# pandekan/tomography_alignment

Hardware: AMD Instinct MI355X
Metric: sirt_iterations_per_sec (higher is better)
Workload: dtype f32

## Files before the change

tomography_alignment_amd/csrc/kernels_tile_gather.hip.h:

```cpp

#define GTX 8
#define GTY 8
#define GROWS 14
#define GPITCH 68
#ifndef GWAVES
#define GWAVES 4
#endif
#ifndef GPX
#define GPX 8
#define GPY 12
#endif

struct GfC {
    int64_t fp0x, fp0y, fux, fuy, fdx, fdy;
    float m00, m01, m10, m11;
    float p0x, p0y, tau;
    int32_t n, zc, slot;
};

__global__ __launch_bounds__(256) void k_sino_zflags(const float *__restrict__ proj, long long n_rows, int ndz, unsigned char *__restrict__ flags)
{
    const int iz = (int)(blockIdx.x * 256 + threadIdx.x);
    if (iz >= ndz) return;
    bool nz = false;
    for (long long r = blockIdx.y; r < n_rows; r += gridDim.y) nz |= proj[(size_t)r * ndz + iz] != 0.f;
    if (nz) flags[iz] = 1;
}

__global__ __launch_bounds__(1024) void k_zflags_prefix(const unsigned char *__restrict__ flags, int n, int *__restrict__ cum)
{
    __shared__ int wsum[16];
    __shared__ int base;
    const int lane = threadIdx.x & 63, wv = threadIdx.x >> 6;
    if (threadIdx.x == 0) base = 0;
    __syncthreads();
    for (int i0 = 0; i0 < n; i0 += 1024) {
        const int i = i0 + (int)threadIdx.x;
        const bool f = i < n && flags[i] != 0;
        const unsigned long long m = __builtin_amdgcn_ballot_w64(f);
        if (lane == 0) wsum[wv] = (int)__builtin_popcountll(m);
        __syncthreads();
        int off = base;
        for (int w = 0; w < wv; ++w) off += wsum[w];
        if (i < n) cum[i] = off + (int)__builtin_popcountll(m & ((1ull << lane) - 1ull));
        __syncthreads();
        if (threadIdx.x == 0) {
            int t = 0;
            for (int w = 0; w < 16; ++w) t += wsum[w];
            base += t;
        }
        __syncthreads();
    }
    if (threadIdx.x == 0) cum[n] = base;
}

__global__ __launch_bounds__(64) void k_zchunk_shift(const unsigned char *__restrict__ flags, int ndz, int nz, int zc_lo, int zc_hi, int *__restrict__ shift)
{
    const int n_chunk = (nz + 63) / 64;
    int first = n_chunk;
    for (int c = threadIdx.x; c < n_chunk; c += 64) {
        bool any = false;
        for (int i = max(0, 64 * c - zc_hi - 1); i <= min(ndz - 1, 64 * c + 63 - zc_lo) && !any; ++i) any = flags[i] != 0;
        if (any) first = min(first, c);
    }
#pragma unroll
    for (int o = 32; o > 0; o >>= 1) first = min(first, __shfl_xor(first, o, 64));
    if (threadIdx.x == 0) *shift = first >= n_chunk ? 0 : (GWAVES - first % GWAVES) % GWAVES;
}

template <bool ZERO>
__device__ __forceinline__ void gather_update_store(float *__restrict__ dst, const float *__restrict__ vv, const float *__restrict__ gt, const f32x2 (&acc2)[32],
                                                    int z0, int nz, int positivity, double *__restrict__ err_out)
{
    double err = 0.0;
#define G_UPD1(R, A, V, G)                                  \
    {                                                       \
        float pr_ = (A) * (V);                              \
        asm volatile("" : "+v"(pr_));        \
        R = R + pr_;                                        \
        if (positivity && R < 0.f) R = 0.f;                 \
        if (gt) { const float e_ = (G) - R; err += (double)e_ * (double)e_; } \
    }
    if (z0 + 64 <= nz && (nz & 3) == 0) {
#pragma unroll
        for (int p = 0; p < 64; p += 4) {
            float4 r = *(float4 *)(dst + p);
            const float4 v = *(const float4 *)(vv + p);
            float4 t = {0.f, 0.f, 0.f, 0.f};
            if (gt) t = *(const float4 *)(gt + p);
            G_UPD1(r.x, ZERO ? 0.f : acc2[p / 2].x, v.x, t.x)
            G_UPD1(r.y, ZERO ? 0.f : acc2[p / 2].y, v.y, t.y)
            G_UPD1(r.z, ZERO ? 0.f : acc2[p / 2 + 1].x, v.z, t.z)
            G_UPD1(r.w, ZERO ? 0.f : acc2[p / 2 + 1].y, v.w, t.w)
            *(float4 *)(dst + p) = r;
            __builtin_amdgcn_sched_barrier(0);
        }
    } else {
#pragma unroll
        for (int p = 0; p < 64; ++p)
            if (z0 + p < nz) {
                float r = dst[p];
                G_UPD1(r, ZERO ? 0.f : ((p & 1) ? acc2[p / 2].y : acc2[p / 2].x), vv[p], gt[p])
                dst[p] = r;
            }
    }
#undef G_UPD1
    if (gt) {
        err = wave_sum_d(err);
        if ((threadIdx.x & 63) == 0) atomicAdd(err_out, err);
    }
}

template <int NJ, int UPD>
__global__ __launch_bounds__(GWAVES * 64, 16 / GWAVES) void k_adj_gather_flat(const GfC *__restrict__ cs, int n_proj, const float *__restrict__ proj,
                                                                 float *__restrict__ vol, TomoGeomC g, int xs, int xe, int patched,
                                                                 const unsigned char *__restrict__ zflags, int zc_lo, int zc_hi, const int *__restrict__ zshift,
                                                                 const float *__restrict__ upd_v, const float *__restrict__ upd_gt, int positivity,
                                                                 double *__restrict__ upd_err)
{
    __shared__ __attribute__((aligned(16))) float rows[GWAVES][GROWS * GPITCH];
    __shared__ float4 wtab[3][GWAVES][64];
    const int lane = threadIdx.x & 63;
    const int wv = __builtin_amdgcn_readfirstlane(threadIdx.x >> 6);
    const int ntx = (xe - xs + GTX - 1) / GTX, nty = (g.ny + GTY - 1) / GTY, nzq = (g.nz + 64 * GWAVES - 1) / (64 * GWAVES) + 1;
    int tx, ty, zq;
    if (patched) {
        const int npx = (ntx + GPX - 1) / GPX, npy = (nty + GPY - 1) / GPY;
        const int slot = (int)(blockIdx.x >> 3), patch = (slot / (GPX * GPY)) * 8 + (int)(blockIdx.x & 7), within = slot % (GPX * GPY);
        const int pxy = patch % (npx * npy);
        zq = patch / (npx * npy);
        tx = (pxy / npy) * GPX + within / GPY;
        ty = (pxy % npy) * GPY + within % GPY;
    } else {
        zq = (int)(blockIdx.x % (unsigned)nzq);
        ty = (int)((blockIdx.x / (unsigned)nzq) % (unsigned)nty);
        tx = (int)(blockIdx.x / ((unsigned)nzq * (unsigned)nty));
    }
    const int x0 = xs + tx * GTX, y0 = ty * GTY, z0 = (zq * GWAVES + wv - *zshift) * 64;
    if (tx >= ntx || ty >= nty || zq >= nzq) return;
    bool zlive = z0 >= 0 && z0 < g.nz;
    if (zlive) {
        bool any = false;
        for (int i = z0 - zc_hi - 1 + lane; i <= z0 + 63 - zc_lo; i += 64) any |= i >= 0 && i < g.ndz && zflags[i] != 0;
        zlive = __builtin_amdgcn_ballot_w64(any) != 0;
    }
    __shared__ int wlive[GWAVES];
    if (lane == 0) wlive[wv] = zlive ? 1 : 0;
    __syncthreads();
    int nl = 0, rk = 0;
#pragma unroll
    for (int w = 0; w < GWAVES; ++w) { nl += wlive[w]; rk += w < wv ? wlive[w] : 0; }
#if !defined(__gfx950__) && !defined(__gfx942__) && !defined(__gfx90a__) && defined(__HIP_DEVICE_COMPILE__)
#error "k_adj_gather_flat: divergent exit before barriers is only known to be safe on gfx9-family targets (s_barrier ignores ended waves)"
#endif
    if (UPD && !zlive && z0 >= 0 && z0 < g.nz && (positivity || upd_gt)) {
        const int X = x0 + (lane >> 3), Y = y0 + (lane & 7);
        if (X < xe && Y < g.ny) {
            const size_t o = ((size_t)X * g.ny + Y) * g.nz + z0;
            f32x2 none[32];
            gather_update_store<true>(vol + o, upd_v + o, upd_gt ? upd_gt + o : nullptr, none, z0, g.nz, positivity, upd_err);
        }
    }
    if (!zlive) return;
    const int X = x0 + (lane >> 3), Y = y0 + (lane & 7), Zl = z0 + lane;
    float *wrows = rows[wv];
    const size_t n_det = (size_t)g.ndx * g.ndz;
    const uint32_t pitch4 = (uint32_t)g.ndz * 4u;
    const float two_m32 = 2.3283064365386963e-10f;
    f32x2 acc2[32];
#pragma unroll
    for (int p = 0; p < 32; ++p) acc2[p] = f32x2{0.f, 0.f};

#define G_TABLE(IPX, BUF, SLOT)                                                                                            \
    {                                                                                                                      \
        float4 t4 = {0.f, 0.f, 0.f, 0.f};                                                                                  \
        if ((IPX) < n_proj) {                                                                                              \
            const GfC &ct = cs[IPX];                                                                                       \
            const float qx = (float)X - ct.p0x, qy = (float)Y - ct.p0y;                                                    \
            const float a = ct.m00 * qx + ct.m01 * qy, b = ct.m10 * qx + ct.m11 * qy;                                      \
            const int i0 = (int)ceilf(a - (fabsf(ct.m00) + fabsf(ct.m01) + 5e-3f));                                        \
            const int j0 = (int)ceilf(b - (fabsf(ct.m10) + fabsf(ct.m11) + 5e-3f));                                        \
            int64_t rx = ct.fp0x + (int64_t)i0 * ct.fux + (int64_t)j0 * ct.fdx - ((int64_t)X << 32);                       \
            int64_t ry = ct.fp0y + (int64_t)i0 * ct.fuy + (int64_t)j0 * ct.fdy - ((int64_t)Y << 32);                       \
            float W[3];                                                                                                    \
            _Pragma("unroll") for (int k = 0; k < 3; ++k) {                                                                \
                int64_t sx = rx, sy = ry;                                                                                  \
                float wsum = 0.f;                                                                                          \
                _Pragma("unroll") for (int mth = 0; mth < NJ; ++mth) {                                                     \
                    const int hx = (int)(sx >> 32), hy = (int)(sy >> 32);                                                  \
                    const float fx = (float)(unsigned)sx * two_m32, fy = (float)(unsigned)sy * two_m32;                    \
                                                        \
                    const float wx = select_lanes2(select_lanes(fx, __builtin_amdgcn_ballot_w64(hx == -1)), 1.f - fx, __builtin_amdgcn_ballot_w64(hx == 0)); \
                    const float wy = select_lanes2(select_lanes(fy, __builtin_amdgcn_ballot_w64(hy == -1)), 1.f - fy, __builtin_amdgcn_ballot_w64(hy == 0)); \
                    wsum += select_lanes(wx * wy, __builtin_amdgcn_ballot_w64((unsigned)(j0 + mth) < (unsigned)ct.n));     \
                    sx += ct.fdx; sy += ct.fdy;                                                                            \
                }                                                                                                          \
                W[k] = select_lanes(wsum, __builtin_amdgcn_ballot_w64((unsigned)(i0 + k) < (unsigned)g.ndx));              \
                rx += ct.fux; ry += ct.fuy;                                                                                \
            }                                                                                                              \
            t4.x = __builtin_bit_cast(float, i0); t4.y = W[0]; t4.z = W[1]; t4.w = W[2];                                   \
        }                                                                                                                  \
        wtab[BUF][SLOT][lane] = t4;                                                                                        \
    }
    float4 tn;
    int ix_lo_n;
    float y0v[GROWS], yedge = 0.f;
#ifdef TOMO_ABLATE_GATHER_LOADS
#define G_ROW_LOAD(P) __int_as_float(0x3f800000 + (int)(size_t)(P))
#else
#define G_ROW_LOAD(P) (*(const float *)(P))
#endif
#define G_SETUP(IPX, BUF, SLOT)                                                                                            \
    {                                                                                                                      \
        tn = wtab[BUF][SLOT][lane];                                                                                        \
        const int i0s = __builtin_bit_cast(int, tn.x);                                                                     \
        ix_lo_n = __builtin_amdgcn_readfirstlane(wave_min_i32(i0s));                                                       \
        if (zlive) {                                                                                                       \
            const GfC &cn = cs[IPX];                                                                                       \
            const int iz0 = Zl - cn.zc;                                                                                    \
            const char *srow = (const char *)(proj + (size_t)cn.slot * n_det);                           \
             \
             \
             \
             \
            const uint32_t o0 = (uint32_t)min(max(iz0, 0), g.ndz - 1) * 4u;                                                 \
            const uint32_t rowoff = (uint32_t)min(max(ix_lo_n + min(lane, GROWS - 1), 0), g.ndx - 1) * pitch4;              \
            _Pragma("unroll") for (int r = 0; r < GROWS; ++r)                                                              \
                y0v[r] = G_ROW_LOAD(srow + (o0 + (uint32_t)__builtin_amdgcn_readlane((int)rowoff, r)));                     \
             \
             \
            if (cn.tau != 0.f) {                                             \
                const uint32_t oe = (uint32_t)min(max(z0 - cn.zc - 1, 0), g.ndz - 1) * 4u;                                  \
                yedge = *(const float *)(srow + (rowoff + oe));                                                            \
            }                                                                                                              \
        }                                                                                                                  \
    }
    const int n_grp = (n_proj + nl - 1) / nl;
    int buf = 0;
    if (n_grp > 0) {
        G_TABLE(rk, 0, rk)
        __syncthreads();
        G_SETUP(0, 0, 0)
    }
    for (int grp = 0; grp < n_grp; ++grp) {
        const int nbuf = buf == 2 ? 0 : buf + 1;
        if (grp + 1 < n_grp) G_TABLE((grp + 1) * nl + rk, nbuf, rk)
        __syncthreads();
        const int g0 = grp * nl, g1 = min(n_proj, g0 + nl);
        for (int ip = g0; ip < g1; ++ip) {
            const GfC &c = cs[ip];
            const float4 t = tn;
            const int i0 = __builtin_bit_cast(int, t.x), ix_lo = ix_lo_n;
            const float W0 = t.y, W1 = t.z, W2 = t.w;
            const bool hit = zlive && __any(W0 != 0.f || W1 != 0.f || W2 != 0.f);
            if (hit) {
                const int iz0 = Zl - c.zc, iz1 = iz0 - 1;
                const unsigned long long m0 = __builtin_amdgcn_ballot_w64(iz0 >= 0) & __builtin_amdgcn_ballot_w64(iz0 < g.ndz);
                const unsigned long long m1 = __builtin_amdgcn_ballot_w64(iz1 >= 0) & __builtin_amdgcn_ballot_w64(iz1 < g.ndz);
#define G_ZLERP(MASKED)                                                                                                           \
    _Pragma("unroll") for (int r = 0; r < GROWS; ++r) {                                                                           \
        float y1 = dpp_shr1_f(y0v[r]);                                             \
        asm("v_writelane_b32 %0, %1, 0" : "+v"(y1) : "s"(__builtin_amdgcn_readlane(__builtin_bit_cast(int, yedge), r)));    \
        const float a0 = (MASKED) ? select_lanes(y0v[r], m0) : y0v[r], a1 = (MASKED) ? select_lanes(y1, m1) : y1;                \
        wrows[r * GPITCH + lane] = fmaf(c.tau, a1 - a0, a0);                                                                      \
    }
                if (c.tau == 0.f) {
                    if (m0 == ~0ull) {
#pragma unroll
                        for (int r = 0; r < GROWS; ++r) wrows[r * GPITCH + lane] = y0v[r];
                    } else {
#pragma unroll
                        for (int r = 0; r < GROWS; ++r) wrows[r * GPITCH + lane] = select_lanes(y0v[r], m0);
                    }
                }
                else if ((m0 & m1) == ~0ull) { G_ZLERP(false) }
                else { G_ZLERP(true) }
#undef G_ZLERP
            }
            if (ip + 1 < g1) G_SETUP(ip + 1, buf, ip + 1 - g0)
            else if (ip + 1 < n_proj) G_SETUP(ip + 1, nbuf, 0)
            if (hit) {
                const int slot0 = min(max(i0 - ix_lo, 0), GROWS - 3);
                const float4 *q = (const float4 *)__builtin_assume_aligned(wrows + slot0 * GPITCH, 16);
                float4 n0 = q[0], n1 = q[GPITCH / 4], n2 = q[2 * GPITCH / 4];
#pragma unroll
                for (int p = 0; p < 64; p += 4) {
                    const float4 r0 = n0, r1 = n1, r2 = n2;
                    if (p + 4 < 64) { n0 = q[(p + 4) / 4]; n1 = q[(GPITCH + p + 4) / 4]; n2 = q[(2 * GPITCH + p + 4) / 4]; }
                    acc2[p / 2] = W2 * f32x2{r2.x, r2.y} + (W1 * f32x2{r1.x, r1.y} + (W0 * f32x2{r0.x, r0.y} + acc2[p / 2]));
                    acc2[p / 2 + 1] = W2 * f32x2{r2.z, r2.w} + (W1 * f32x2{r1.z, r1.w} + (W0 * f32x2{r0.z, r0.w} + acc2[p / 2 + 1]));
                    __builtin_amdgcn_sched_barrier(0);
                }
            }
        }
        buf = nbuf;
    }
#undef G_TABLE
#undef G_SETUP
    if (UPD) {
        if (X < xe && Y < g.ny) {
            const size_t o = ((size_t)X * g.ny + Y) * g.nz + z0;
            gather_update_store<false>(vol + o, upd_v + o, upd_gt ? upd_gt + o : nullptr, acc2, z0, g.nz, positivity, upd_err);
        }
    } else if (zlive && X < xe && Y < g.ny) {
        float *dst = vol + ((size_t)X * g.ny + Y) * g.nz + z0;
        if (z0 + 64 <= g.nz && (g.nz & 3) == 0) {
#pragma unroll
            for (int p = 0; p < 64; p += 4) {
                float4 v = *(float4 *)(dst + p);
                v.x += acc2[p / 2].x; v.y += acc2[p / 2].y; v.z += acc2[p / 2 + 1].x; v.w += acc2[p / 2 + 1].y;
                *(float4 *)(dst + p) = v;
            }
        } else {
#pragma unroll
            for (int p = 0; p < 64; ++p)
                if (z0 + p < g.nz) dst[p] += (p & 1) ? acc2[p / 2].y : acc2[p / 2].x;
        }
    }
}


#define FGROWS 24
#define FG_NONE (1 << 29)

template <int NW, int WALKY>
__device__ __forceinline__ void fwd_gather_flat_body(const GfC *__restrict__ cs, const int *__restrict__ perm, int n_list, unsigned block_id,
                                                     float *__restrict__ proj, const float *__restrict__ vol, const TomoGeomC &g,
                                                     const unsigned char *__restrict__ vflags, const int *__restrict__ zshift,
                                                     float (*rows)[FGROWS * GPITCH], float4 (*wtab)[GWAVES][64], int (*ltab)[GWAVES][64], int *wlive)
{
    static_assert(NW == 3 || NW == 4, "NW");
    constexpr int SW = FGROWS - NW + 1;
    const int lane = threadIdx.x & 63;
    const int wv = __builtin_amdgcn_readfirstlane(threadIdx.x >> 6);
    const int nS = WALKY ? g.ny : g.nx, nL = WALKY ? g.nx : g.ny;
    const uint32_t strideL4 = (WALKY ? (uint32_t)g.ny * (uint32_t)g.nz : (uint32_t)g.nz) * 4u;
    const size_t strideS = WALKY ? (size_t)g.nz : (size_t)g.ny * g.nz;
    const int npg = (n_list + 7) / 8, nrt = (g.ndx + 7) / 8, nzq = (g.nz + 64 * GWAVES - 1) / (64 * GWAVES) + 1;
    const int m_all = npg * nrt, m8 = (m_all + 7) / 8;
    const int slot_id = (int)(block_id >> 3), xcd = (int)(block_id & 7);
    const int zq = slot_id / m8, tile = xcd * m8 + slot_id % m8;
    if (tile >= m_all || zq >= nzq) return;
    const int pg = tile / nrt, rt = tile % nrt;
    const int z0 = (zq * GWAVES + wv - *zshift) * 64;
    bool zlive = z0 >= 0 && z0 < g.nz;
    if (zlive) {
        const int i = z0 + lane;
        zlive = __builtin_amdgcn_ballot_w64(i < g.nz && vflags[i] != 0) != 0;
    }
    if (lane == 0) wlive[wv] = zlive ? 1 : 0;
    __syncthreads();
    int nl = 0, rk = 0;
#pragma unroll
    for (int w = 0; w < GWAVES; ++w) { nl += wlive[w]; rk += w < wv ? wlive[w] : 0; }
#if !defined(__gfx950__) && !defined(__gfx942__) && !defined(__gfx90a__) && defined(__HIP_DEVICE_COMPILE__)
#error "k_fwd_gather_flat: divergent exit before barriers is only known to be safe on gfx9-family targets (s_barrier ignores ended waves)"
#endif
    if (!zlive) return;

    const int ipl = pg * 8 + (lane >> 3), ix = rt * 8 + (lane & 7);
    const int pe = perm[min(ipl, n_list - 1)];
    const bool ray_ok = ipl < n_list && ix < g.ndx && pe >= 0;
    const GfC &c = cs[max(pe, 0)];
    const int64_t fds = WALKY ? c.fdy : c.fdx, fdl = WALKY ? c.fdx : c.fdy;
    const int64_t bs0 = (WALKY ? c.fp0y : c.fp0x) + (int64_t)ix * (WALKY ? c.fuy : c.fux);
    const int64_t bl0 = (WALKY ? c.fp0x : c.fp0y) + (int64_t)ix * (WALKY ? c.fux : c.fuy);
    const float bsf = (float)((double)bs0 * 2.3283064365386963e-10), inv_ds = (float)(4294967296.0 / (double)fds);
    const int n_smp = ray_ok ? c.n : 0;
    const float two_m32 = 2.3283064365386963e-10f;
    const int Zl = z0 + lane;
    const unsigned long long mz = __builtin_amdgcn_ballot_w64(Zl < g.nz);
    const uint32_t o0 = (uint32_t)min(Zl, g.nz - 1) * 4u;
    float *wrows = rows[wv];
    f32x2 acc2[32];
#pragma unroll
    for (int p = 0; p < 32; ++p) acc2[p] = f32x2{0.f, 0.f};

#define FG_TABLE(SX, BUF, SLOT)                                                                                            \
    {                                                                                                                      \
        float W[4] = {0.f, 0.f, 0.f, 0.f};                                                                                 \
        int L0 = FG_NONE;                                                                                                  \
        if ((SX) < nS) {                                                                                                   \
            const float ta = ((float)((SX) - 1) - bsf) * inv_ds, tb = ((float)((SX) + 1) - bsf) * inv_ds;                  \
            const int j0 = (int)ceilf(fminf(ta, tb) - 5e-3f);                                                              \
            int64_t sx = bs0 + (int64_t)j0 * fds - ((int64_t)(SX) << 32), sl = bl0 + (int64_t)j0 * fdl;                    \
            float wx[3], fl[3];                                                                                            \
            int hl[3];                                                                                                     \
            _Pragma("unroll") for (int mth = 0; mth < 3; ++mth) {                                                          \
                const int hx = (int)(sx >> 32);                                                                            \
                const float fx = (float)(unsigned)sx * two_m32;                                                            \
                float w = hx == -1 ? fx : (hx == 0 ? 1.f - fx : 0.f);                                                      \
                w = (unsigned)(j0 + mth) < (unsigned)n_smp ? w : 0.f;                                                      \
                wx[mth] = w;                                                                                               \
                hl[mth] = (int)(sl >> 32);                                                                                 \
                fl[mth] = (float)(unsigned)sl * two_m32;                                                                   \
                if (w > 0.f) L0 = min(L0, hl[mth]);                                                                        \
                sx += fds; sl += fdl;                                                                                      \
            }                                                                                                              \
            _Pragma("unroll") for (int mth = 0; mth < 3; ++mth) {                                                          \
                const int rel = hl[mth] - L0;                                                                              \
                const float wl1 = wx[mth] * fl[mth], wl0 = wx[mth] - wl1;                                                  \
                _Pragma("unroll") for (int k = 0; k < NW; ++k) W[k] += rel == k ? wl0 : (rel == k - 1 ? wl1 : 0.f);        \
            }                                                                                                              \
            bool any = false;                                                                                              \
            _Pragma("unroll") for (int k = 0; k < NW; ++k) {                                                               \
                W[k] = (unsigned)(L0 + k) < (unsigned)nL ? W[k] : 0.f;                                                     \
                any |= W[k] != 0.f;                                                                                        \
            }                                                                                                              \
            if (!any) L0 = FG_NONE;                                                                                        \
        }                                                                                                                  \
        wtab[BUF][SLOT][lane] = make_float4(W[0], W[1], W[2], W[3]);                                                       \
        ltab[BUF][SLOT][lane] = L0;                                                                                        \
    }
    float4 tn;
    int Ln, Llo_n, Lhi_n, need_n = 0;
    float yv[FGROWS];
#define FG_SETUP(SX, BUF, SLOT)                                                                                            \
    {                                                                                                                      \
        tn = wtab[BUF][SLOT][lane];                                                                                        \
        Ln = ltab[BUF][SLOT][lane];                                                                                        \
        Llo_n = __builtin_amdgcn_readfirstlane(wave_min_i32(Ln));                                                          \
        Lhi_n = __builtin_amdgcn_readfirstlane(wave_max_i32(Ln == FG_NONE ? -FG_NONE : Ln));                               \
        if (Llo_n != FG_NONE) {                                                                                            \
            const char *sbase = (const char *)(vol + (size_t)(SX) * strideS);                            \
            const uint32_t lineoff = (uint32_t)min(max(Llo_n + min(lane, FGROWS - 1), 0), nL - 1) * strideL4;              \
                    \
            need_n = min(Lhi_n - Llo_n + NW, FGROWS);                                                                      \
            _Pragma("unroll") for (int r4 = 0; r4 < FGROWS; r4 += 4)                                                       \
                if (r4 < need_n) {                                                                                         \
                    _Pragma("unroll") for (int r = r4; r < r4 + 4; ++r)                                                    \
                        yv[r] = *(const float *)(sbase + (o0 + (uint32_t)__builtin_amdgcn_readlane((int)lineoff, r)));     \
                }                                                                                                          \
        }                                                                                                                  \
    }
#define FG_ACCUM(LBASE)                                                                                                    \
    {                                                                                                                      \
        const int rel = L - (LBASE);                                                                                       \
        const bool inw = (unsigned)rel < (unsigned)SW;                                                                     \
        const int slot0 = inw ? rel : 0;                                                                                   \
        const float W0 = inw ? t.x : 0.f, W1 = inw ? t.y : 0.f, W2 = inw ? t.z : 0.f, W3 = inw ? t.w : 0.f;                \
        const float4 *q = (const float4 *)__builtin_assume_aligned(wrows + slot0 * GPITCH, 16);                            \
        float4 n0 = q[0], n1 = q[GPITCH / 4], n2 = q[2 * GPITCH / 4], n3 = {0.f, 0.f, 0.f, 0.f};                           \
        if (NW == 4) n3 = q[3 * GPITCH / 4];                                                                               \
        _Pragma("unroll") for (int p = 0; p < 64; p += 4) {                                                                \
            const float4 r0 = n0, r1 = n1, r2 = n2, r3 = n3;                                                               \
            if (p + 4 < 64) {                                                                                              \
                n0 = q[(p + 4) / 4]; n1 = q[(GPITCH + p + 4) / 4]; n2 = q[(2 * GPITCH + p + 4) / 4];                       \
                if (NW == 4) n3 = q[(3 * GPITCH + p + 4) / 4];                                                             \
            }                                                                                                              \
            f32x2 a = W2 * f32x2{r2.x, r2.y} + (W1 * f32x2{r1.x, r1.y} + (W0 * f32x2{r0.x, r0.y} + acc2[p / 2]));          \
            f32x2 b = W2 * f32x2{r2.z, r2.w} + (W1 * f32x2{r1.z, r1.w} + (W0 * f32x2{r0.z, r0.w} + acc2[p / 2 + 1]));      \
            if (NW == 4) { a = W3 * f32x2{r3.x, r3.y} + a; b = W3 * f32x2{r3.z, r3.w} + b; }                               \
            acc2[p / 2] = a; acc2[p / 2 + 1] = b;                                                                          \
            __builtin_amdgcn_sched_barrier(0);                                                                             \
        }                                                                                                                  \
    }
    const int n_grp = (nS + nl - 1) / nl;
    int buf = 0;
    FG_TABLE(rk, 0, rk)
    __syncthreads();
    FG_SETUP(0, 0, 0)
    for (int grp = 0; grp < n_grp; ++grp) {
        const int nbuf = buf == 2 ? 0 : buf + 1;
        if (grp + 1 < n_grp) FG_TABLE((grp + 1) * nl + rk, nbuf, rk)
        __syncthreads();
        const int g0 = grp * nl, g1 = min(nS, g0 + nl);
        for (int sx = g0; sx < g1; ++sx) {
            const float4 t = tn;
            const int L = Ln, Llo = Llo_n, Lhi = Lhi_n, need = need_n;
            const bool hit = Llo != FG_NONE;
            if (hit) {
                if (mz == ~0ull) {
#pragma unroll
                    for (int r4 = 0; r4 < FGROWS; r4 += 4)
                        if (r4 < need) {
#pragma unroll
                            for (int r = r4; r < r4 + 4; ++r) wrows[r * GPITCH + lane] = yv[r];
                        }
                } else {
#pragma unroll
                    for (int r4 = 0; r4 < FGROWS; r4 += 4)
                        if (r4 < need) {
#pragma unroll
                            for (int r = r4; r < r4 + 4; ++r) wrows[r * GPITCH + lane] = select_lanes(yv[r], mz);
                        }
                }
            }
            if (sx + 1 < g1) FG_SETUP(sx + 1, buf, sx + 1 - g0)
            else if (sx + 1 < nS) FG_SETUP(sx + 1, nbuf, 0)
            if (hit) {
                FG_ACCUM(Llo)
                for (int lb = Llo + SW; lb <= Lhi; lb += SW) {
                    const char *sbase = (const char *)(vol + (size_t)sx * strideS);
                    for (int r = 0; r < FGROWS; r += 4) {
                        float e[4];
#pragma unroll
                        for (int k = 0; k < 4; ++k)
                            e[k] = *(const float *)(sbase + (o0 + (uint32_t)min(max(lb + r + k, 0), nL - 1) * strideL4));
#pragma unroll
                        for (int k = 0; k < 4; ++k) wrows[(r + k) * GPITCH + lane] = select_lanes(e[k], mz);
                    }
                    FG_ACCUM(lb)
                }
            }
        }
        buf = nbuf;
    }
#undef FG_TABLE
#undef FG_SETUP
#undef FG_ACCUM
    if (!ray_ok) return;
    const int iz0 = z0 - c.zc;
    float *dst = proj + (size_t)c.slot * ((size_t)g.ndx * g.ndz) + (size_t)ix * g.ndz + iz0;
    const float tau = c.tau;
    if (tau == 0.f) {
        if (iz0 >= 0 && iz0 + 64 <= g.ndz && ((iz0 | g.ndz) & 3) == 0) {
#pragma unroll
            for (int p = 0; p < 64; p += 4) *(float4 *)(dst + p) = make_float4(acc2[p / 2].x, acc2[p / 2].y, acc2[p / 2 + 1].x, acc2[p / 2 + 1].y);
        } else {
#pragma unroll
            for (int p = 0; p < 64; ++p)
                if ((unsigned)(iz0 + p) < (unsigned)g.ndz) dst[p] = (p & 1) ? acc2[p / 2].y : acc2[p / 2].x;
        }
    } else {
        const float wfz = 1.f - tau;
#define FG_S(P) (((P) & 1) ? acc2[(P) / 2].y : acc2[(P) / 2].x)
#pragma unroll
        for (int p = 0; p < 63; ++p)
            if ((unsigned)(iz0 + p) < (unsigned)g.ndz) dst[p] = wfz * FG_S(p) + tau * FG_S(p + 1);
        if ((unsigned)(iz0 + 63) < (unsigned)g.ndz) atomicAdd(dst + 63, wfz * FG_S(63));
        if ((unsigned)(iz0 - 1) < (unsigned)g.ndz) atomicAdd(dst - 1, tau * FG_S(0));
#undef FG_S
    }
}

__global__ __launch_bounds__(GWAVES * 64, 3) void k_fwd_gather_flat(const GfC *__restrict__ cs, const int *__restrict__ perm, int n0, int n1, int n2, int n3,
                                                                    float *__restrict__ proj, const float *__restrict__ vol, TomoGeomC g,
                                                                    const unsigned char *__restrict__ vflags, const int *__restrict__ zshift)
{
    __shared__ __attribute__((aligned(16))) float rows[GWAVES][FGROWS * GPITCH];
    __shared__ float4 wtab[3][GWAVES][64];
    __shared__ int ltab[3][GWAVES][64];
    __shared__ int wlive[GWAVES];
    const unsigned nrt = (unsigned)(g.ndx + 7) / 8, nzq = (unsigned)(g.nz + 64 * GWAVES - 1) / (64 * GWAVES) + 1;
    const unsigned w0 = 8u * ((((unsigned)n0 + 7) / 8 * nrt + 7) / 8) * nzq, w1 = 8u * ((((unsigned)n1 + 7) / 8 * nrt + 7) / 8) * nzq,
                   w2 = 8u * ((((unsigned)n2 + 7) / 8 * nrt + 7) / 8) * nzq;
    unsigned b = blockIdx.x;
    if (b < w0) { fwd_gather_flat_body<3, 0>(cs, perm, n0, b, proj, vol, g, vflags, zshift, rows, wtab, ltab, wlive); return; }
    b -= w0;
    if (b < w1) { fwd_gather_flat_body<4, 0>(cs, perm + n0, n1, b, proj, vol, g, vflags, zshift, rows, wtab, ltab, wlive); return; }
    b -= w1;
    if (b < w2) { fwd_gather_flat_body<3, 1>(cs, perm + n0 + n1, n2, b, proj, vol, g, vflags, zshift, rows, wtab, ltab, wlive); return; }
    b -= w2;
    fwd_gather_flat_body<4, 1>(cs, perm + n0 + n1 + n2, n3, b, proj, vol, g, vflags, zshift, rows, wtab, ltab, wlive);
}
```

Before: 3.431.

## Use buffer loads, DPP wave reductions, and restage gather pipeline in tile kernels

Replaces the global-pointer row loads in both the backprojection and forward-projection gather kernels with raw buffer loads, using a per-row or per-slab resource descriptor so scalar offsets can be passed directly. Replaces the wave min/max helpers with DPP-based reductions plus four readlanes. Restructures the per-projection loop so the next item's loads are issued first, the current item's accumulate runs while they are in flight, and the LDS staging of the next rows happens afterwards. Buffer-load bounds checking also changes out-of-range behaviour. The zlive guard on the loads is removed, so some loads that were skipped before may now be issued.

```diff
diff --git a/tomography_alignment_amd/csrc/kernels_tile_gather.hip.h b/tomography_alignment_amd/csrc/kernels_tile_gather.hip.h
--- a/tomography_alignment_amd/csrc/kernels_tile_gather.hip.h
+++ b/tomography_alignment_amd/csrc/kernels_tile_gather.hip.h
@@ -10,6 +10,25 @@
 #define GPX 8
 #define GPY 12
 #endif
+
+#define G_DPP(V, CTRL) __builtin_amdgcn_update_dpp(0, (V), (CTRL), 0xf, 0xf, true)
+__device__ __forceinline__ int gwave_min_i32(int v)
+{
+    v = min(v, G_DPP(v, 0xB1));
+    v = min(v, G_DPP(v, 0x4E));
+    v = min(v, G_DPP(v, 0x141));
+    v = min(v, G_DPP(v, 0x140));
+    return min(min(__builtin_amdgcn_readlane(v, 0), __builtin_amdgcn_readlane(v, 16)), min(__builtin_amdgcn_readlane(v, 32), __builtin_amdgcn_readlane(v, 48)));
+}
+__device__ __forceinline__ int gwave_max_i32(int v)
+{
+    v = max(v, G_DPP(v, 0xB1));
+    v = max(v, G_DPP(v, 0x4E));
+    v = max(v, G_DPP(v, 0x141));
+    v = max(v, G_DPP(v, 0x140));
+    return max(max(__builtin_amdgcn_readlane(v, 0), __builtin_amdgcn_readlane(v, 16)), max(__builtin_amdgcn_readlane(v, 32), __builtin_amdgcn_readlane(v, 48)));
+}
+#undef G_DPP
 
 struct GfC {
     int64_t fp0x, fp0y, fux, fuy, fdx, fdy;
@@ -202,45 +221,71 @@
         }                                                                                                                  \
         wtab[BUF][SLOT][lane] = t4;                                                                                        \
     }
-    float4 tn;
-    int ix_lo_n;
-    float y0v[GROWS], yedge = 0.f;
 #ifdef TOMO_ABLATE_GATHER_LOADS
-#define G_ROW_LOAD(P) __int_as_float(0x3f800000 + (int)(size_t)(P))
+#define G_ROW_LOAD(RS, VOFF, SOFF) __int_as_float(0x3f800000 + (int)((VOFF) + (SOFF)))
 #else
-#define G_ROW_LOAD(P) (*(const float *)(P))
+#define G_ROW_LOAD(RS, VOFF, SOFF) __builtin_bit_cast(float, __builtin_amdgcn_raw_buffer_load_b32((RS), (VOFF), (SOFF), 0))
 #endif
+    const uint32_t det_bytes = (uint32_t)min((unsigned long long)n_det * 4ull, 0xffffffffull);
 #define G_SETUP(IPX, BUF, SLOT)                                                                                            \
     {                                                                                                                      \
         tn = wtab[BUF][SLOT][lane];                                                                                        \
         const int i0s = __builtin_bit_cast(int, tn.x);                                                                     \
-        ix_lo_n = __builtin_amdgcn_readfirstlane(wave_min_i32(i0s));                                                       \
-        if (zlive) {                                                                                                       \
-            const GfC &cn = cs[IPX];                                                                                       \
-            const int iz0 = Zl - cn.zc;                                                                                    \
-            const char *srow = (const char *)(proj + (size_t)cn.slot * n_det);                           \
-             \
-             \
-             \
-             \
-            const uint32_t o0 = (uint32_t)min(max(iz0, 0), g.ndz - 1) * 4u;                                                 \
-            const uint32_t rowoff = (uint32_t)min(max(ix_lo_n + min(lane, GROWS - 1), 0), g.ndx - 1) * pitch4;              \
-            _Pragma("unroll") for (int r = 0; r < GROWS; ++r)                                                              \
-                y0v[r] = G_ROW_LOAD(srow + (o0 + (uint32_t)__builtin_amdgcn_readlane((int)rowoff, r)));                     \
-             \
-             \
-            if (cn.tau != 0.f) {                                             \
-                const uint32_t oe = (uint32_t)min(max(z0 - cn.zc - 1, 0), g.ndz - 1) * 4u;                                  \
-                yedge = *(const float *)(srow + (rowoff + oe));                                                            \
+        ix_lo_n = __builtin_amdgcn_readfirstlane(gwave_min_i32(i0s));                                                      \
+        const GfC &cn = cs[IPX];                                                                                           \
+        const int iz0 = Zl - cn.zc;                                                                                        \
+        const __amdgpu_buffer_rsrc_t srs =                                                                                 \
+            __builtin_amdgcn_make_buffer_rsrc((void *)(proj + (size_t)cn.slot * n_det), 0, (int)det_bytes, 0x00020000);    \
+        const uint32_t o0 = (uint32_t)min(max(iz0, 0), g.ndz - 1) * 4u;                                                    \
+        const uint32_t rowoff = (uint32_t)min(max(ix_lo_n + min(lane, GROWS - 1), 0), g.ndx - 1) * pitch4;                 \
+        _Pragma("unroll") for (int r = 0; r < GROWS; ++r)                                                                  \
+            y0v[r] = G_ROW_LOAD(srs, o0, (uint32_t)__builtin_amdgcn_readlane((int)rowoff, r));                             \
+         \
+         \
+        if (cn.tau != 0.f) {                                                 \
+            const uint32_t oe = (uint32_t)min(max(z0 - cn.zc - 1, 0), g.ndz - 1) * 4u;                                     \
+            yedge = __builtin_bit_cast(float, __builtin_amdgcn_raw_buffer_load_b32(srs, rowoff + oe, 0, 0));               \
+        }                                                                                                                  \
+    }
+#define G_ZLERP(MASKED, TAU)                                                                                                      \
+    _Pragma("unroll") for (int r = 0; r < GROWS; ++r) {                                                                           \
+        float y1 = dpp_shr1_f(y0v[r]);                                             \
+        asm("v_writelane_b32 %0, %1, 0" : "+v"(y1) : "s"(__builtin_amdgcn_readlane(__builtin_bit_cast(int, yedge), r)));    \
+        const float a0 = (MASKED) ? select_lanes(y0v[r], m0) : y0v[r], a1 = (MASKED) ? select_lanes(y1, m1) : y1;                \
+        wrows[r * GPITCH + lane] = fmaf((TAU), a1 - a0, a0);                                                                      \
+    }
+#define G_STAGE(IPX)                                                                                                       \
+    {                                                                                                                      \
+        const GfC &cn = cs[IPX];                                                                                           \
+        const int iz0 = Zl - cn.zc, iz1 = iz0 - 1;                                                                         \
+        const unsigned long long m0 = __builtin_amdgcn_ballot_w64(iz0 >= 0) & __builtin_amdgcn_ballot_w64(iz0 < g.ndz);    \
+        const unsigned long long m1 = __builtin_amdgcn_ballot_w64(iz1 >= 0) & __builtin_amdgcn_ballot_w64(iz1 < g.ndz);    \
+        if (cn.tau == 0.f) {             \
+            if (m0 == ~0ull) {           \
+                _Pragma("unroll") for (int r = 0; r < GROWS; ++r) wrows[r * GPITCH + lane] = y0v[r];     \
+            } else {                                                                                                       \
+                _Pragma("unroll") for (int r = 0; r < GROWS; ++r) wrows[r * GPITCH + lane] = select_lanes(y0v[r], m0);     \
             }                                                                                                              \
         }                                                                                                                  \
-    }
+        else if ((m0 & m1) == ~0ull) { G_ZLERP(false, cn.tau) }      \
+        else { G_ZLERP(true, cn.tau) }                                                                                     \
+    }
+#define G_HIT(T) (__any((T).y != 0.f || (T).z != 0.f || (T).w != 0.f))
     const int n_grp = (n_proj + nl - 1) / nl;
     int buf = 0;
+    float4 t = {0.f, 0.f, 0.f, 0.f};
+    int ix_lo = 0;
+    bool hit = false;
     if (n_grp > 0) {
         G_TABLE(rk, 0, rk)
         __syncthreads();
+        float4 tn;
+        int ix_lo_n;
+        float y0v[GROWS], yedge = 0.f;
         G_SETUP(0, 0, 0)
+        hit = G_HIT(tn);
+        if (hit) G_STAGE(0)
+        t = tn; ix_lo = ix_lo_n;
     }
     for (int grp = 0; grp < n_grp; ++grp) {
         const int nbuf = buf == 2 ? 0 : buf + 1;
@@ -248,38 +293,18 @@
         __syncthreads();
         const int g0 = grp * nl, g1 = min(n_proj, g0 + nl);
         for (int ip = g0; ip < g1; ++ip) {
-            const GfC &c = cs[ip];
-            const float4 t = tn;
-            const int i0 = __builtin_bit_cast(int, t.x), ix_lo = ix_lo_n;
-            const float W0 = t.y, W1 = t.z, W2 = t.w;
-            const bool hit = zlive && __any(W0 != 0.f || W1 != 0.f || W2 != 0.f);
+            float4 tn = t;
+            int ix_lo_n = ix_lo;
+            float y0v[GROWS], yedge = 0.f;
+            const bool more = ip + 1 < n_proj;
+            if (more) {
+                const bool same = ip + 1 < g1;
+                const int sbuf = same ? buf : nbuf, sslot = same ? ip + 1 - g0 : 0;
+                G_SETUP(ip + 1, sbuf, sslot)
+            }
             if (hit) {
-                const int iz0 = Zl - c.zc, iz1 = iz0 - 1;
-                const unsigned long long m0 = __builtin_amdgcn_ballot_w64(iz0 >= 0) & __builtin_amdgcn_ballot_w64(iz0 < g.ndz);
-                const unsigned long long m1 = __builtin_amdgcn_ballot_w64(iz1 >= 0) & __builtin_amdgcn_ballot_w64(iz1 < g.ndz);
-#define G_ZLERP(MASKED)                                                                                                           \
-    _Pragma("unroll") for (int r = 0; r < GROWS; ++r) {                                                                           \
-        float y1 = dpp_shr1_f(y0v[r]);                                             \
-        asm("v_writelane_b32 %0, %1, 0" : "+v"(y1) : "s"(__builtin_amdgcn_readlane(__builtin_bit_cast(int, yedge), r)));    \
-        const float a0 = (MASKED) ? select_lanes(y0v[r], m0) : y0v[r], a1 = (MASKED) ? select_lanes(y1, m1) : y1;                \
-        wrows[r * GPITCH + lane] = fmaf(c.tau, a1 - a0, a0);                                                                      \
-    }
-                if (c.tau == 0.f) {
-                    if (m0 == ~0ull) {
-#pragma unroll
-                        for (int r = 0; r < GROWS; ++r) wrows[r * GPITCH + lane] = y0v[r];
-                    } else {
-#pragma unroll
-                        for (int r = 0; r < GROWS; ++r) wrows[r * GPITCH + lane] = select_lanes(y0v[r], m0);
-                    }
-                }
-                else if ((m0 & m1) == ~0ull) { G_ZLERP(false) }
-                else { G_ZLERP(true) }
-#undef G_ZLERP
-            }
-            if (ip + 1 < g1) G_SETUP(ip + 1, buf, ip + 1 - g0)
-            else if (ip + 1 < n_proj) G_SETUP(ip + 1, nbuf, 0)
-            if (hit) {
+                const int i0 = __builtin_bit_cast(int, t.x);
+                const float W0 = t.y, W1 = t.z, W2 = t.w;
                 const int slot0 = min(max(i0 - ix_lo, 0), GROWS - 3);
                 const float4 *q = (const float4 *)__builtin_assume_aligned(wrows + slot0 * GPITCH, 16);
                 float4 n0 = q[0], n1 = q[GPITCH / 4], n2 = q[2 * GPITCH / 4];
@@ -292,11 +317,18 @@
                     __builtin_amdgcn_sched_barrier(0);
                 }
             }
+            hit = more && G_HIT(tn);
+            if (hit) G_STAGE(ip + 1)
+            t = tn; ix_lo = ix_lo_n;
         }
         buf = nbuf;
     }
 #undef G_TABLE
+#undef G_ROW_LOAD
 #undef G_SETUP
+#undef G_ZLERP
+#undef G_STAGE
+#undef G_HIT
     if (UPD) {
         if (X < xe && Y < g.ny) {
             const size_t o = ((size_t)X * g.ny + Y) * g.nz + z0;
@@ -412,24 +444,40 @@
         wtab[BUF][SLOT][lane] = make_float4(W[0], W[1], W[2], W[3]);                                                       \
         ltab[BUF][SLOT][lane] = L0;                                                                                        \
     }
-    float4 tn;
-    int Ln, Llo_n, Lhi_n, need_n = 0;
-    float yv[FGROWS];
+    const uint32_t slab_bytes = (uint32_t)min(WALKY ? (unsigned long long)(g.nx - 1) * strideL4 + (unsigned long long)g.nz * 4ull
+                                                    : (unsigned long long)g.ny * g.nz * 4ull, 0xffffffffull);
+#define FG_SLAB_RSRC(SX) __builtin_amdgcn_make_buffer_rsrc((void *)(vol + (size_t)(SX) * strideS), 0, (int)slab_bytes, 0x00020000)
+#define FG_LINE_LOAD(RS, SOFF) __builtin_bit_cast(float, __builtin_amdgcn_raw_buffer_load_b32((RS), o0, (SOFF), 0))
 #define FG_SETUP(SX, BUF, SLOT)                                                                                            \
     {                                                                                                                      \
         tn = wtab[BUF][SLOT][lane];                                                                                        \
         Ln = ltab[BUF][SLOT][lane];                                                                                        \
-        Llo_n = __builtin_amdgcn_readfirstlane(wave_min_i32(Ln));                                                          \
-        Lhi_n = __builtin_amdgcn_readfirstlane(wave_max_i32(Ln == FG_NONE ? -FG_NONE : Ln));                               \
+        Llo_n = __builtin_amdgcn_readfirstlane(gwave_min_i32(Ln));                                                         \
+        Lhi_n = __builtin_amdgcn_readfirstlane(gwave_max_i32(Ln == FG_NONE ? -FG_NONE : Ln));                              \
+        need_n = 0;                                                                                                        \
         if (Llo_n != FG_NONE) {                                                                                            \
-            const char *sbase = (const char *)(vol + (size_t)(SX) * strideS);                            \
+            const __amdgpu_buffer_rsrc_t srs = FG_SLAB_RSRC(SX);                                                           \
             const uint32_t lineoff = (uint32_t)min(max(Llo_n + min(lane, FGROWS - 1), 0), nL - 1) * strideL4;              \
                     \
             need_n = min(Lhi_n - Llo_n + NW, FGROWS);                                                                      \
             _Pragma("unroll") for (int r4 = 0; r4 < FGROWS; r4 += 4)                                                       \
                 if (r4 < need_n) {                                                                                         \
                     _Pragma("unroll") for (int r = r4; r < r4 + 4; ++r)                                                    \
-                        yv[r] = *(const float *)(sbase + (o0 + (uint32_t)__builtin_amdgcn_readlane((int)lineoff, r)));     \
+                        yv[r] = FG_LINE_LOAD(srs, (uint32_t)__builtin_amdgcn_readlane((int)lineoff, r));                   \
+                }                                                                                                          \
+        }                                                                                                                  \
+    }
+#define FG_STAGE                                                                                                           \
+    {                                                                                                                      \
+        if (mz == ~0ull) {                                                                                                 \
+            _Pragma("unroll") for (int r4 = 0; r4 < FGROWS; r4 += 4)                                                       \
+                if (r4 < need_n) {                                                                                         \
+                    _Pragma("unroll") for (int r = r4; r < r4 + 4; ++r) wrows[r * GPITCH + lane] = yv[r];                  \
+                }                                                                                                          \
+        } else {                                                                                                           \
+            _Pragma("unroll") for (int r4 = 0; r4 < FGROWS; r4 += 4)                                                       \
+                if (r4 < need_n) {                                                                                         \
+                    _Pragma("unroll") for (int r = r4; r < r4 + 4; ++r) wrows[r * GPITCH + lane] = select_lanes(yv[r], mz); \
                 }                                                                                                          \
         }                                                                                                                  \
     }
@@ -459,55 +507,54 @@
     int buf = 0;
     FG_TABLE(rk, 0, rk)
     __syncthreads();
-    FG_SETUP(0, 0, 0)
+    float4 t;
+    int L, Llo, Lhi;
+    {
+        float4 tn;
+        int Ln, Llo_n, Lhi_n, need_n;
+        float yv[FGROWS];
+        FG_SETUP(0, 0, 0)
+        FG_STAGE
+        t = tn; L = Ln; Llo = Llo_n; Lhi = Lhi_n;
+    }
     for (int grp = 0; grp < n_grp; ++grp) {
         const int nbuf = buf == 2 ? 0 : buf + 1;
         if (grp + 1 < n_grp) FG_TABLE((grp + 1) * nl + rk, nbuf, rk)
         __syncthreads();
         const int g0 = grp * nl, g1 = min(nS, g0 + nl);
         for (int sx = g0; sx < g1; ++sx) {
-            const float4 t = tn;
-            const int L = Ln, Llo = Llo_n, Lhi = Lhi_n, need = need_n;
-            const bool hit = Llo != FG_NONE;
-            if (hit) {
-                if (mz == ~0ull) {
-#pragma unroll
-                    for (int r4 = 0; r4 < FGROWS; r4 += 4)
-                        if (r4 < need) {
-#pragma unroll
-                            for (int r = r4; r < r4 + 4; ++r) wrows[r * GPITCH + lane] = yv[r];
-                        }
-                } else {
-#pragma unroll
-                    for (int r4 = 0; r4 < FGROWS; r4 += 4)
-                        if (r4 < need) {
-#pragma unroll
-                            for (int r = r4; r < r4 + 4; ++r) wrows[r * GPITCH + lane] = select_lanes(yv[r], mz);
-                        }
-                }
+            float4 tn = t;
+            int Ln = L, Llo_n = FG_NONE, Lhi_n = 0, need_n = 0;
+            float yv[FGROWS];
+            if (sx + 1 < nS) {
+                const bool same = sx + 1 < g1;
+                const int sbuf = same ? buf : nbuf, sslot = same ? sx + 1 - g0 : 0;
+                FG_SETUP(sx + 1, sbuf, sslot)
             }
-            if (sx + 1 < g1) FG_SETUP(sx + 1, buf, sx + 1 - g0)
-            else if (sx + 1 < nS) FG_SETUP(sx + 1, nbuf, 0)
-            if (hit) {
+            if (Llo != FG_NONE) {
                 FG_ACCUM(Llo)
                 for (int lb = Llo + SW; lb <= Lhi; lb += SW) {
-                    const char *sbase = (const char *)(vol + (size_t)sx * strideS);
+                    const __amdgpu_buffer_rsrc_t srs = FG_SLAB_RSRC(sx);
                     for (int r = 0; r < FGROWS; r += 4) {
                         float e[4];
 #pragma unroll
-                        for (int k = 0; k < 4; ++k)
-                            e[k] = *(const float *)(sbase + (o0 + (uint32_t)min(max(lb + r + k, 0), nL - 1) * strideL4));
+                        for (int k = 0; k < 4; ++k) e[k] = FG_LINE_LOAD(srs, (uint32_t)min(max(lb + r + k, 0), nL - 1) * strideL4);
 #pragma unroll
                         for (int k = 0; k < 4; ++k) wrows[(r + k) * GPITCH + lane] = select_lanes(e[k], mz);
                     }
                     FG_ACCUM(lb)
                 }
             }
+            FG_STAGE
+            t = tn; L = Ln; Llo = Llo_n; Lhi = Lhi_n;
         }
         buf = nbuf;
     }
 #undef FG_TABLE
+#undef FG_SLAB_RSRC
+#undef FG_LINE_LOAD
 #undef FG_SETUP
+#undef FG_STAGE
 #undef FG_ACCUM
     if (!ray_ok) return;
     const int iz0 = z0 - c.zc;
```

Measured after the change: 3.716, median of 6. 1.08x the previous value.
